# yifita/iso-points

Hardware: AMD Instinct MI355X
Metric: Mpoints/s full iso-point cycle (project+resample+splat), 1M pts (higher is better)
Workload: dtype f32-class (split-fp16 operands, 2^-22: hidden-layer products from two fp16 parts per f32 operand under exact power-of-two scales, 3 fp16-MFMA passes, f32 accumulate; everything else f32)

## Files before the change

### include/isopoints.h

```cpp
#ifndef ISOPOINTS_H_
#define ISOPOINTS_H_

#include <stdint.h>

#ifdef __cplusplus
extern "C" {
#endif

#define ISO_OK 0
#define ISO_ERR_INVALID (-1)
#define ISO_ERR_UNSUPPORTED (-2)
#define ISO_ERR_LAUNCH (-3)
#define ISO_ERR_WORKSPACE (-4)

const char* iso_version(void);
const char* iso_last_error(void);


int iso_project_sphere(const float* pts_in, float* pts_out, float* normals_out,
                       uint8_t* mask_out, int64_t n, float cx, float cy,
                       float cz, float radius, int max_iters, float tol,
                       void* stream);

typedef struct iso_follow {
  void* grid_ws; int64_t grid_n_max;
  const float* views; int n_views; float znear; float zfar; int backface_culling;
  int32_t* mask_out; void* front_ws; int64_t front_ws_bytes;
  int64_t* first_idx_out; int64_t* num_pts_out; int32_t* view_total_out;
} iso_follow;

int iso_project_sphere_follow(const float* pts_in, float* pts_out, float* normals_out,
                              uint8_t* mask_out, int64_t n, float cx, float cy,
                              float cz, float radius, int max_iters, float tol,
                              const iso_follow* follow_host, void* stream);

int64_t iso_siren_raw_floats(int hidden, int n_hidden);
int64_t iso_siren_packed_floats(int hidden, int n_hidden);
int iso_siren_pack_weights(const float* raw, float* packed, int hidden,
                           int n_hidden, void* stream);
int iso_siren_set_gemm_mode(int mode);
int iso_siren_get_gemm_mode(void);
int iso_siren_set_tail_from(int first_tail_iteration);
int iso_siren_set_drawn_tiles(int on);
int iso_idr_set_drawn_tiles(int on);
int iso_siren_step_launches(int hidden, int n_hidden, int max_iters);
int64_t iso_project_siren_workspace_bytes(int64_t n, int hidden, int n_hidden);
int64_t iso_project_siren_counts_offset(int64_t n, int hidden, int n_hidden);
int iso_project_siren(const float* pts_in, float* pts_out, float* normals_out,
                      uint8_t* mask_out, int64_t n, const float* packed,
                      int hidden, int n_hidden, float omega_first,
                      float omega_hidden, int max_iters, float tol,
                      void* workspace, int64_t workspace_bytes, void* stream);
int iso_siren_sdf_grad(const float* pts, float* sdf_out, float* grad_out,
                       int64_t n, const float* packed, int hidden,
                       int n_hidden, float omega_first, float omega_hidden,
                       void* workspace, int64_t workspace_bytes, void* stream);

int iso_siren_fold_codes(const float* w0c, const float* b0, const float* codes, float* table, int hidden,
                         int padded_hidden, int c_dim, int64_t n_codes, void* stream);
int iso_project_siren_coded(const float* pts_in, float* pts_out, float* normals_out,
                            uint8_t* mask_out, int64_t n, const float* packed,
                            int hidden, int n_hidden, float omega_first,
                            float omega_hidden, int max_iters, float tol,
                            void* workspace, int64_t workspace_bytes, void* stream,
                            const float* code_bias, const int32_t* code_of, int64_t n_codes);
int iso_siren_sdf_grad_coded(const float* pts, float* sdf_out, float* grad_out,
                             int64_t n, const float* packed, int hidden,
// ... 449 lines not shown
```

### iso_points_amd/_lib.py

```python
import ctypes
import os

import torch

_HERE = os.path.dirname(os.path.abspath(__file__))
LIB_PATH = os.path.join(_HERE, "libisopoints_hip.so")
if os.environ.get("ISO_DEV_LIB"):
    LIB_PATH = os.path.abspath(os.environ["ISO_DEV_LIB"])

_c = ctypes
_P = _c.c_void_p
_I = _c.c_int
_L = _c.c_int64
_F = _c.c_float

SIGNATURES = {
    "iso_version": (_c.c_char_p, []),
    "iso_last_error": (_c.c_char_p, []),
    "iso_project_sphere": (_I, [_P, _P, _P, _P, _L, _F, _F, _F, _F, _I, _F, _P]),
    "iso_project_sphere_follow": (_I, [_P, _P, _P, _P, _L, _F, _F, _F, _F, _I, _F, _P, _P]),
    "iso_siren_raw_floats": (_L, [_I, _I]),
    "iso_siren_packed_floats": (_L, [_I, _I]),
    "iso_siren_set_gemm_mode": (_I, [_I]),
    "iso_siren_get_gemm_mode": (_I, []),
    "iso_siren_set_tail_from": (_I, [_I]),
    "iso_siren_set_drawn_tiles": (_I, [_I]),
    "iso_idr_set_drawn_tiles": (_I, [_I]),
    "iso_siren_step_launches": (_I, [_I, _I, _I]),
    "iso_siren_pack_weights": (_I, [_P, _P, _I, _I, _P]),
    "iso_project_siren_workspace_bytes": (_L, [_L, _I, _I]),
    "iso_project_siren_counts_offset": (_L, [_L, _I, _I]),
    "iso_project_siren": (_I, [_P, _P, _P, _P, _L, _P, _I, _I, _F, _F, _I, _F, _P, _L, _P]),
    "iso_siren_sdf_grad": (_I, [_P, _P, _P, _L, _P, _I, _I, _F, _F, _P, _L, _P]),
    "iso_idr_set_gemm_mode": (_I, [_I]),
    "iso_idr_get_gemm_mode": (_I, []),
    "iso_idr_step_form": (_I, [_I, _I, _I, _I, _I]),
    "iso_idr_raw_floats": (_L, [_I, _I, _I, _I]),
    "iso_idr_packed_floats": (_L, [_I, _I]),
    "iso_idr_pack_weights": (_I, [_P, _P, _I, _I, _I, _I, _P]),
    "iso_project_idr_workspace_bytes": (_L, [_L, _I, _I]),
    "iso_project_idr": (_I, [_P, _P, _P, _P, _L, _P, _I, _I, _I, _I, _F, _I, _F, _P, _L, _P]),
    "iso_idr_sdf_grad": (_I, [_P, _P, _P, _L, _P, _I, _I, _I, _I, _F, _P, _L, _P]),
    "iso_trace_sphere": (_I, [_P, _P, _P, _P, _P, _L, _F, _F, _F, _F, _F, _F, _I, _F, _P]),
    "iso_trace_siren": (_I, [_P, _P, _P, _P, _P, _L, _P, _I, _I, _F, _F, _F, _F, _I, _F, _P, _L, _P]),
    "iso_siren_fold_codes": (_I, [_P, _P, _P, _P, _I, _I, _I, _L, _P]),
    "iso_project_siren_coded": (_I, [_P, _P, _P, _P, _L, _P, _I, _I, _F, _F, _I, _F, _P, _L, _P, _P, _P, _L]),
    "iso_siren_sdf_grad_coded": (_I, [_P, _P, _P, _L, _P, _I, _I, _F, _F, _P, _L, _P, _P, _P, _L]),
    "iso_trace_siren_coded": (_I, [_P, _P, _P, _P, _P, _L, _P, _I, _I, _F, _F, _F, _F, _I, _F, _P, _L, _P, _P, _P, _L]),
    "iso_trace_idr": (_I, [_P, _P, _P, _P, _P, _L, _P, _I, _I, _I, _I, _F, _F, _F, _I, _F, _P, _L, _P]),
    "iso_ray_nearest_point_workspace_bytes": (_L, [_L]),
# ... 181 lines not shown
```

### iso_points_amd/csrc/siren.hip

```cpp
#include <stdlib.h>
#include "siren_common.h"
#include "iso_newton.h"
#include "mlp_common.h"

namespace {

__global__ void k_siren_pack(const float* __restrict__ raw, float* __restrict__ packed,
                             int H, int L) {
  const int64_t total = off_hidden(H, L);
  const int64_t HH = (int64_t)H * H;
  const int NT = H / 16;
  for (int64_t o = (int64_t)blockIdx.x * blockDim.x + threadIdx.x; o < total;
       o += (int64_t)gridDim.x * blockDim.x) {
    float v = 0.f;
    if (o < off_wl(H)) {
      int64_t k = o;
      int c = (int)(k & 3);
      int e = (int)((k >> 2) % (H / 4));
      int g = (int)((k >> 2) / (H / 4));
      int f = 16 * (e >> 2) + 4 * g + (e & 3);
      v = (c < 3) ? raw[f * 3 + c] : raw[(int64_t)H * 3 + f];
    } else if (o < off_bl(H)) {
      int64_t k = o - off_wl(H);
      int e = (int)(k % (H / 4));
// ... 265 lines not shown
static int64_t tail_ints(int64_t n) { return siren_x3_tail_blocks() * (2 * tail_cap_of(n) + 2); }

constexpr int kTileCtrInts = 128;
extern "C" int64_t iso_project_siren_workspace_bytes(int64_t n, int hidden, int n_hidden) {
  if (n < 0) n = 0;
  return stash_floats_any(hidden, n_hidden) * 4 + 2 * n * 4 + tail_ints(n) * 4 + (64 + kTileCtrInts) * 4 + 64;
}

extern "C" int64_t iso_project_siren_counts_offset(int64_t n, int hidden, int n_hidden) {
  if (n < 0) n = 0;
  return stash_floats_any(hidden, n_hidden) * 4 + 2 * n * 4 + tail_ints(n) * 4;
}

static int g_siren_dyn_tiles = -1;
static bool siren_dynamic_tiles_enabled() {
  return g_siren_dyn_tiles != 0;
}
extern "C" int iso_siren_set_drawn_tiles(int on) {
  ISO_REQUIRE(on >= -1 && on <= 1, ISO_ERR_INVALID, "iso_siren_set_drawn_tiles: -1 (default), 0 or 1");
  g_siren_dyn_tiles = on;
  return ISO_OK;
}

static int run_step_split(SirenCodedArgs a, int hidden, int64_t n, hipStream_t s) {
  if (hidden == 256 && !a.fwd_only && use_x3(hidden, a.L)) {
    a.split = 3;
    return run_step(a, hidden, n, s);
  }
  a.split = 0;
  a.tile_ctr = nullptr;
  return run_step(a, hidden, n, s);
}

static int g_tail_from = -1;
static int siren_tail_from(int max_iters) {
  if (g_tail_from == 0) return max_iters + 1;
  if (g_tail_from > 0) return g_tail_from;
  return max_iters >= 6 ? 4 : 2;
}
extern "C" int iso_siren_step_launches(int hidden, int n_hidden, int max_iters) {
  if (max_iters < 0) return 0;
  const bool can_tail = hidden == 256 && use_x3(hidden, n_hidden);
  const int from = can_tail ? siren_tail_from(max_iters) : max_iters + 1;
  return from <= max_iters && from > 0 ? from + 1 : max_iters + 1;
}
extern "C" int iso_siren_set_tail_from(int first_tail_iteration) {
// ... 235 lines not shown
```

### iso_points_amd/csrc/siren_common.h

```cpp
#pragma once
#include "iso_common.h"

struct SirenArgs {
  float* pts;
  float* normals;
  uint8_t* mask;
  float* sdf_out;
  float* grad_out;
  const int32_t* idx_in;
  const int32_t* count_in;
  int32_t* idx_out;
  int32_t* count_out;
  const float* packed;
  float* stash;
  int64_t n;
  int L;
  float w0, wh, tol;
  int do_move;
  int eval_only;
  const float* dirs = nullptr;
  float alpha = 1.f, bound = 0.f, tol_valid = 0.f;
  int fwd_only = 0;
  int64_t cnt_lo = -1, cnt_hi = INT64_MAX;
  int small_tiles = 0;
// ... 28 lines not shown
__host__ __device__ inline int64_t off_hidden(int H, int l) {
  return 5 * (int64_t)H + 4 + (int64_t)l * ((int64_t)H + 2 * (int64_t)H * H);
}

__host__ __device__ inline int x3_feat(int s, int kappa) {
  return 32 * (s >> 1) + 16 * (s & 1) + 8 * ((kappa & 7) >> 2) + 4 * (kappa >> 3) + (kappa & 3);
}
__host__ __device__ inline int64_t x3_base(int H, int L) { return off_hidden(H, L); }
__host__ __device__ inline int64_t x3_off_w0(int H, int L) { return x3_base(H, L); }
__host__ __device__ inline int64_t x3_off_wl(int H, int L) { return x3_base(H, L) + 4 * (int64_t)H; }
__host__ __device__ inline int64_t x3_off_layer(int H, int L, int l) {
  return x3_base(H, L) + 5 * (int64_t)H + (int64_t)l * (int64_t)H;
}
constexpr int kX16Header = 24;
__host__ __device__ inline int64_t x16_base(int H, int L) { return x3_off_layer(H, L, L); }
__host__ __device__ inline int64_t x16_off_layer(int H, int L, int l) { return x16_base(H, L) + kX16Header + (int64_t)l * H * H; }
__host__ __device__ inline int64_t x16_off_bw(int H, int L, int l) { return x16_off_layer(H, L, L) + (int64_t)l * H * H; }
__host__ __device__ inline int64_t siren_packed_total(int H, int L) { return x16_off_bw(H, L, L); }

bool siren_x3_supported(int H, int L);
int64_t siren_x3_stash_floats(int H, int L);
void siren_x3_pack(const float* raw, float* packed, int H, int L, hipStream_t s);
int siren_x3_launch(const SirenCodedArgs& a, int H, int64_t n_upper, hipStream_t s);
int siren_x3_tail_blocks();
int siren_x3_launch_tail(const SirenCodedArgs& a, int H, hipStream_t s);
constexpr int64_t kPsMinList = 3 * 256 * 128;
__host__ __device__ inline bool siren_ps_takes(int64_t count, int L, const float* hdr , float wh) {
  if (count < kPsMinList) return false;
  float r = 0.f;
  for (int l = 0; l < L; ++l) r = hdr[17 + l] > r ? hdr[17 + l] : r;
  return (wh * r) * 1.01f < 1.0e4f;
}
```

### iso_points_amd/csrc/siren_x3.hip

```cpp
#include <stdlib.h>
#include <type_traits>
#include "siren_common.h"
#include "iso_newton.h"
#include "mlp_common.h"

#include "mfma_split.h"

constexpr int kAD = 3;

namespace {

__device__ __forceinline__ void x3_sin_wcos8(float w_in, float w, const float (&z)[8], float (&s)[8], float (&c)[8]) {
  iso_sin_wcos8(w_in, w, z, s, c);
}


__global__ void k_siren_pack_x3(const float* __restrict__ raw, float* __restrict__ packed, int H, int L) {
  const int64_t base = x3_base(H, L), total = x16_base(H, L);
  const int64_t HH = (int64_t)H * H;
  const float* b0 = raw + (int64_t)H * 3;
  const float* WL = raw + (int64_t)H * 4 + (int64_t)L * (HH + H);
  for (int64_t o = base + (int64_t)blockIdx.x * blockDim.x + threadIdx.x; o < total;
       o += (int64_t)gridDim.x * blockDim.x) {
    const int64_t rel = o - base;
// ... 77 lines not shown
    const bool bwd = o >= (int64_t)L * HH;
    const int l = (int)((o / HH) % L);
    const int64_t q = o % HH;
    const float* Wl = raw + (int64_t)H * 4 + (int64_t)l * (HH + H);
    const float sc = packed[x16_base(H, L) + l];
    const int d = (int)(q & 3), lane = (int)((q >> 2) & 63);
    const int64_t blk = q >> 8;
    const int part = (int)(blk & 1);
    const int To = (int)((blk >> 1) % NTO), s = (int)(blk / (2 * NTO));
    const int fo = 32 * To + (lane & 31);
    f32x2 v;
#pragma unroll
    for (int u = 0; u < 2; ++u) {
      const int fi = x3_feat(s, 8 * (lane >> 5) + 2 * d + u);
      v[u] = (bwd ? Wl[(int64_t)fi * H + fo] : Wl[(int64_t)fo * H + fi]) * sc;
    }
    const f16x2 h = __builtin_convertvector(v, f16x2);
    const f16x2 lo = __builtin_convertvector(v - __builtin_convertvector(h, f32x2), f16x2);
    reinterpret_cast<unsigned*>(packed + x16_off_layer(H, L, 0))[o] =
        part == 0 ? __builtin_bit_cast(unsigned, h) : __builtin_bit_cast(unsigned, lo);
  }
}

template <int H, int NW, int NB>
struct X3Shape {
  static constexpr int NS = H / 16;
  static constexpr int NTO = H / 32;
  static constexpr int TW = NTO / NW;
  static constexpr int SL = 2 * TW;
  static constexpr int NG = SL * NB;
  static constexpr int P = 32 * NB;
  static constexpr size_t kActBytes = (size_t)NS * NB * kAP * 1024;
  static constexpr size_t kRedBytes = (size_t)NW * P * 16;
  static constexpr size_t kPtsBytes = (size_t)P * 16;
  static constexpr int kLdsGroupsFit = (int)((163840 - (kActBytes + kRedBytes + kPtsBytes)) / ((size_t)NW * 2048));
  static constexpr int LG = kLdsGroupsFit < NG ? kLdsGroupsFit : NG;
  static constexpr size_t kLds = kActBytes + kRedBytes + kPtsBytes + (size_t)NW * LG * 2048;
  static constexpr int64_t kStashPerWg(int L) { return (int64_t)NW * (L > 1 ? L : 1) * NG * 512; }
  static_assert(NTO % NW == 0 && TW >= 1, "features must split evenly over the waves");
};

template <int H>
__device__ __forceinline__ void x3_code_bias8(const float* table, int row, int s, int h, float (&b)[8]) {
  const f32x4* t = reinterpret_cast<const f32x4*>(table + (int64_t)row * H + 16 * s + 4 * h);
  const f32x4 lo = t[0], hi = t[2];
#pragma unroll
  for (int e = 0; e < 4; ++e) { b[e] = lo[e]; b[4 + e] = hi[e]; }
}

template <int H, int NW, int NB, bool FWD, bool CODED>
__device__ __forceinline__ void x3_step_body(const typename SirenArgsOf<CODED>::type& a, const int bid, const int nblk,
                                             const int sid) {
  using S = X3Shape<H, NW, NB>;
  constexpr int NS = S::NS, NTO = S::NTO, TW = S::TW, SL = S::SL, NG = S::NG, P = S::P;
  extern __shared__ __attribute__((aligned(16))) unsigned char smem_raw[];
  u32x4* act = reinterpret_cast<u32x4*>(smem_raw);
  f32x4* red = reinterpret_cast<f32x4*>(smem_raw + S::kActBytes);
  f32x4* ptl = reinterpret_cast<f32x4*>(smem_raw + S::kActBytes + S::kRedBytes);
  constexpr int LG = S::LG;
  const int tid = threadIdx.x;
  const int w = __builtin_amdgcn_readfirstlane(tid >> 6);
  const int lane = tid & 63, h = lane >> 5, j = lane & 31;
  u32x4* own = act + (size_t)(SL * w) * NB * kAP * 64 + lane;
  u32x4* park = own + (size_t)(kAP - 2) * NG * 64;
  constexpr bool IL = (NW == 8);
  const int L = a.L;
  const float* X = a.packed + x3_base(H, L);
  const f32x4* W0u = reinterpret_cast<const f32x4*>(X) + SL * w * 16;
  const float* WLu = X + 4 * H + SL * w * 16;
  const int h8 = h * 8;
  const float bL = a.packed[off_bl(H)];
  f32x4* stash = reinterpret_cast<f32x4*>(a.stash) +
                 ((int64_t)sid * NW + w) * (int64_t)(L > 1 ? L : 1) * NG * 128;
  f32x4* lst = reinterpret_cast<f32x4*>(smem_raw + S::kActBytes + S::kRedBytes + S::kPtsBytes) + w * (LG * 128) + lane;

  constexpr int FP = 2, BP = 2;
  auto fwd_img = [&](int l) { return reinterpret_cast<const u32x4*>(a.packed + x16_off_layer(H, L, l)) + (TW * w * 2) * 64; };
  auto rev_img = [&](int l) { return reinterpret_cast<const u32x4*>(a.packed + x16_off_bw(H, L, l)) + (TW * w * 2) * 64; };
  auto fwd_scale = [&](int l) { return kActScale * a.packed[x16_base(H, L) + l]; };
  float* redm = reinterpret_cast<float*>(red);
  float bscale[NB];
  float amax[NB];
  auto put_amax = [&](int buf) {
#pragma unroll
    for (int n = 0; n < NB; ++n) {
      const float m = __builtin_fmaxf(amax[n], __shfl_xor(amax[n], 32));
      if (h == 0) redm[(buf * P + 32 * n + j) * NW + w] = m;
    }
  };
  u32x4 A[4][TW][3];
  x3_prefetch_a<kAD, TW, NTO, FP>(A, fwd_img(0), 0, lane);

  const int64_t total = a.count_in ? (int64_t)__hip_atomic_load(a.count_in, __ATOMIC_RELAXED, __HIP_MEMORY_SCOPE_AGENT) : a.n;
  if (total <= a.cnt_lo || total > a.cnt_hi) return;
  if (a.ps_guard && H == 256 && siren_ps_takes(total, L, a.packed + x16_base(H, L), a.wh)) return;
  const int64_t cut = a.split ? siren_split_point(total) : total;
  const int64_t slot0 = a.split == 2 ? cut : 0;
  const int64_t count = a.split == 1 ? cut : total;
  const int64_t n_tiles = (count - slot0 + P - 1) / P;
  __shared__ int s_next_tile, s_first_tile;
  int nidx[NB];
  float npx[NB], npy[NB], npz[NB];
  int nrow[NB];
  auto fetch_idx = [&](int64_t t) {
    int j_e = j;
    asm volatile("" : "+v"(j_e));
#pragma unroll
    for (int n = 0; n < NB; ++n) {
      const int64_t slot = slot0 + t * P + 32 * n + j_e;
      nidx[n] = -1;
      if (t < n_tiles && slot < count) nidx[n] = a.idx_in ? a.idx_in[slot] : (int)slot;
// ... 48 lines not shown
        float zz[8], hv[8], sv[8];
        if constexpr (CODED) {
          float bz[8];
          x3_code_bias8<H>(a.code_bias, row[n], SL * w + sl, h, bz);
#pragma unroll
          for (int e = 0; e < 8; ++e) zz[e] = ((wv[e].x * px[n] + wv[e].y * py[n]) + wv[e].z * pz[n]) + bz[e];
        } else {
#pragma unroll
          for (int e = 0; e < 8; ++e) zz[e] = ((wv[e].x * px[n] + wv[e].y * py[n]) + wv[e].z * pz[n]) + wv[e].w;
        }
        x3_sin_wcos8(a.w0, a.w0, zz, hv, sv);
        const int k = sl * NB + n;
        {
          u32x4 p0, p1;
          split8_f16(hv, p0, p1);
          own[(k * kAP + 0) * 64] = p0; own[(k * kAP + 1) * 64] = p1;
        }
        (void)sv;
      }
    }
    __syncthreads();

    f32x16 acc[TW][NB];
    float fpart[NB];
#pragma unroll
    for (int n = 0; n < NB; ++n) fpart[n] = 0.f;
    for (int l = 0; l < L; ++l) {
      const float* lay = a.packed + x3_off_layer(H, L, l);
      const u32x4* img = fwd_img(l);
      const float zscale = fwd_scale(l);
      const float w_in = a.wh / zscale;
      if (l + 1 < L || FWD) {
        gemm_x3<kAD, TW, NB, NTO, NS, kBias, IL, FP, FP>(img, lay, act + lane, acc, w, 0, A,
                                                         l + 1 < L ? fwd_img(l + 1) : fwd_img(0), 0, lane, zscale);
      } else {
        gemm_x3<kAD, TW, NB, NTO, NS, kBias, IL, FP, BP>(img, lay, act + lane, acc, w, 0, A, rev_img(L - 1), 0, lane,
                                                         zscale);
      }
      __syncthreads();
      const bool top = (l == L - 1);
      f32x4* st_l = stash + (int64_t)l * NG * 128;
      const bool lds_slot = (l == 0);
      const float seed_scale = x3_scale_for(a.packed[x16_base(H, L) + 16] * a.wh * 1.01f);
      if (top) {
#pragma unroll
        for (int n = 0; n < NB; ++n) { amax[n] = 0.f; bscale[n] = seed_scale; }
      }
      auto act_group = [&](int k, int n, int sl, const float (&zz)[8], float& fp) {
        float hv[8], sv[8];
        x3_sin_wcos8(w_in, a.wh, zz, hv, sv);
        if (top) {
          const f32x4 wl0 = *reinterpret_cast<const f32x4*>(WLu + sl * 16 + h8);
          const f32x4 wl1 = *reinterpret_cast<const f32x4*>(WLu + sl * 16 + h8 + 4);
          const float f0 = (wl0.x * hv[0] + wl0.y * hv[1]) + (wl0.z * hv[2] + wl0.w * hv[3]);
          const float f1 = (wl1.x * hv[4] + wl1.y * hv[5]) + (wl1.z * hv[6] + wl1.w * hv[7]);
          fp += f0 + f1;
          if constexpr (FWD) return;
#pragma unroll
          for (int e = 0; e < 4; ++e) { hv[e] = wl0[e] * sv[e]; hv[4 + e] = wl1[e] * sv[4 + e]; }
          float m = amax[n];
#pragma unroll
          for (int e = 0; e < 8; e += 2) m = __builtin_fmaxf(m, __builtin_fmaxf(__builtin_fabsf(hv[e]), __builtin_fabsf(hv[e + 1])));
          amax[n] = m;
          u32x4 p0, p1;
          split8_f16(hv, p0, p1, seed_scale);
          own[(k * kAP + 0) * 64] = p0; own[(k * kAP + 1) * 64] = p1;
          return;
        } else {
          if constexpr (!FWD) {
            if (k < LG && lds_slot) {
              lst[(k * 2 + 0) * 64] = (f32x4){sv[0], sv[1], sv[2], sv[3]};
              lst[(k * 2 + 1) * 64] = (f32x4){sv[4], sv[5], sv[6], sv[7]};
            } else {
              st_l[(k * 2 + 0) * 64 + lane] = (f32x4){sv[0], sv[1], sv[2], sv[3]};
              st_l[(k * 2 + 1) * 64 + lane] = (f32x4){sv[4], sv[5], sv[6], sv[7]};
            }
          }
        }
        u32x4 p0, p1;
        split8_f16(hv, p0, p1);
        own[(k * kAP + 0) * 64] = p0; own[(k * kAP + 1) * 64] = p1;
      };
      if constexpr (NG <= 8) {
#pragma unroll
        for (int t = 0; t < TW; ++t)
#pragma unroll
          for (int p = 0; p < 2; ++p)
#pragma unroll
            for (int n = 0; n < NB; ++n) {
              float zz[8];
#pragma unroll
              for (int e = 0; e < 8; ++e) zz[e] = acc[t][n][8 * p + e];
              act_group((2 * t + p) * NB + n, n, 2 * t + p, zz, fpart[n]);
              __builtin_amdgcn_sched_barrier(0);
            }
      } else {
#pragma unroll
        for (int t = 0; t < TW; ++t)
#pragma unroll
          for (int n = 0; n < NB; ++n)
#pragma unroll
            for (int p = 0; p < 2; ++p) {
              const int k = (2 * t + p) * NB + n;
              const f32x16& v = acc[t][n];
              park[(k * 2 + 0) * 64] = as_u32x4((f32x4){v[8 * p], v[8 * p + 1], v[8 * p + 2], v[8 * p + 3]});
              park[(k * 2 + 1) * 64] = as_u32x4((f32x4){v[8 * p + 4], v[8 * p + 5], v[8 * p + 6], v[8 * p + 7]});
            }
        for (int sl = 0; sl < SL; ++sl) {
          f32x4 z[NB][2];
#pragma unroll
          for (int n = 0; n < NB; ++n) {
            z[n][0] = as_f32x4(park[((sl * NB + n) * 2 + 0) * 64]);
            z[n][1] = as_f32x4(park[((sl * NB + n) * 2 + 1) * 64]);
          }
#pragma unroll
          for (int n = 0; n < NB; ++n) {
            float zz[8];
#pragma unroll
            for (int e = 0; e < 8; ++e) zz[e] = z[n][e >> 2][e & 3];
            act_group(sl * NB + n, n, sl, zz, fpart[n]);
          }
        }
      }
      if constexpr (!FWD) { if (top) put_amax(0); }
      __syncthreads();
    }
    float gx[NB], gy[NB], gz[NB];
#pragma unroll
    for (int n = 0; n < NB; ++n) gx[n] = gy[n] = gz[n] = 0.f;
    int mbuf = 0;
    auto get_amax = [&](float (&Mp)[NB]) {
#pragma unroll
      for (int n = 0; n < NB; ++n) {
        float m = 0.f;
#pragma unroll
        for (int ww = 0; ww < NW; ++ww) m = __builtin_fmaxf(m, redm[(mbuf * P + 32 * n + j) * NW + ww]);
        Mp[n] = m;
      }
    };
    for (int l = FWD ? 0 : L - 1; l >= 1; --l) {
      const u32x4* img = rev_img(l);
      const f32x4* st_l = stash + (int64_t)(l - 1) * NG * 128;
      f32x4 sv[NG][2];
      auto ld_stash = [&]() {
#pragma unroll
        for (int k = 0; k < NG; ++k) {
          if (k < LG && l == 1) {
            sv[k][0] = lst[(k * 2) * 64]; sv[k][1] = lst[(k * 2 + 1) * 64];
          } else {
            sv[k][0] = st_l[(k * 2) * 64 + lane]; sv[k][1] = st_l[(k * 2 + 1) * 64 + lane];
          }
        }
      };
      float Mp[NB];
      get_amax(Mp);
      gemm_x3<kAD, TW, NB, NTO, NS, kZero, IL, BP, BP>(img, nullptr, act + lane, acc, w, 0, A, rev_img(l - 1), 0, lane);
      ld_stash();
      __syncthreads();
      float inv[NB], nscale[NB];
      {
        const float iw = 1.0f / a.packed[x16_base(H, L) + l];
        const float grow = a.packed[x16_base(H, L) + 8 + l] * a.wh * 1.01f;
#pragma unroll
        for (int n = 0; n < NB; ++n) {
          inv[n] = iw / bscale[n];
          nscale[n] = x3_scale_for(Mp[n] * grow);
          amax[n] = 0.f;
        }
      }
#pragma unroll
      for (int t = 0; t < TW; ++t)
#pragma unroll
        for (int p = 0; p < 2; ++p) {
#pragma unroll
          for (int n = 0; n < NB; ++n) {
            const int k = (2 * t + p) * NB + n;
            float av[8];
#pragma unroll
            for (int e = 0; e < 8; ++e) av[e] = (acc[t][n][8 * p + e] * inv[n]) * sv[k][e >> 2][e & 3];
            float m = amax[n];
#pragma unroll
            for (int e = 0; e < 8; e += 2) m = __builtin_fmaxf(m, __builtin_fmaxf(__builtin_fabsf(av[e]), __builtin_fabsf(av[e + 1])));
            amax[n] = m;
            u32x4 p0, p1;
            split8_f16(av, p0, p1, nscale[n]);
            own[(k * kAP + 0) * 64] = p0; own[(k * kAP + 1) * 64] = p1;
          }
        }
#pragma unroll
      for (int n = 0; n < NB; ++n) bscale[n] = nscale[n];
      put_amax(mbuf ^ 1);
      mbuf ^= 1;
      __syncthreads();
    }
    if constexpr (!FWD) {
      int drawn = 0;
      if (dyn && tid == 0) drawn = draw_base + atomicAdd(a.tile_ctr, 1);
      gemm_x3<kAD, TW, NB, NTO, NS, kZero, IL, BP, FP>(rev_img(0), nullptr, act + lane, acc, w, 0, A, fwd_img(0), 0, lane);
      if (dyn && tid == 0) s_next_tile = drawn;
      __syncthreads();
      next_tile = dyn ? (int64_t)s_next_tile : tile + nblk;
      fetch_idx(next_tile);
      float inv[NB];
      {
        const float iw = 1.0f / a.packed[x16_base(H, L)];
#pragma unroll
        for (int n = 0; n < NB; ++n) inv[n] = iw / bscale[n];
      }
      f32x4 q[NB];
#pragma unroll
      for (int n = 0; n < NB; ++n) q[n] = ptl[32 * n + j];
#pragma unroll
      for (int t = 0; t < TW; ++t)
#pragma unroll
        for (int p = 0; p < 2; ++p) {
          f32x4 wv[8];
#pragma unroll
          for (int e = 0; e < 8; ++e) wv[e] = W0u[(2 * t + p) * 16 + h8 + e];
#pragma unroll
          for (int n = 0; n < NB; ++n) {
            float zz[8], cv[8];
            if constexpr (CODED) {
              float bz[8];
              x3_code_bias8<H>(a.code_bias, __float_as_int(q[n].w), SL * w + 2 * t + p, h, bz);
#pragma unroll
              for (int e = 0; e < 8; ++e) zz[e] = ((wv[e].x * q[n].x + wv[e].y * q[n].y) + wv[e].z * q[n].z) + bz[e];
            } else {
#pragma unroll
              for (int e = 0; e < 8; ++e) zz[e] = ((wv[e].x * q[n].x + wv[e].y * q[n].y) + wv[e].z * q[n].z) + wv[e].w;
            }
            iso_wcos8(a.w0, a.w0, zz, cv);
#pragma unroll
            for (int e = 0; e < 8; ++e) {
              const float av = (acc[t][n][8 * p + e] * inv[n]) * cv[e];
              gx[n] += wv[e].x * av;
              gy[n] += wv[e].y * av;
              gz[n] += wv[e].z * av;
            }
            __builtin_amdgcn_sched_barrier(0);
          }
        }
    } else {
      next_tile = tile + nblk;
      fetch_idx(next_tile);
    }
#pragma unroll
    for (int n = 0; n < NB; ++n) {
      float f = fpart[n] + __shfl_xor(fpart[n], 32);
      float x = gx[n] + __shfl_xor(gx[n], 32);
      float y = gy[n] + __shfl_xor(gy[n], 32);
      float z = gz[n] + __shfl_xor(gz[n], 32);
      if (h == 0) red[w * P + 32 * n + j] = (f32x4){f, x, y, z};
    }
    int tid_e = tid, lane_e = lane;
    asm volatile("" : "+v"(tid_e), "+v"(lane_e));
    int eidx = -1;
    f32x4 qe = {0.f, 0.f, 0.f, 0.f};
    {
      const int64_t slot = slot0 + tile * P + tid_e;
      if (tid_e < P && slot < count) {
        eidx = a.idx_in ? a.idx_in[slot] : (int)slot;
        if constexpr (!FWD) qe = ptl[tid_e];
      }
      fetch_pts();
    }
    __syncthreads();
    bool survive = false;
    int64_t idx = -1;
    {
      const int64_t slot = slot0 + tile * P + tid_e;
      if (tid_e < P && slot < count) {
        f32x4 r = red[tid_e];
#pragma unroll
        for (int ww = 1; ww < NW; ++ww) {
          const f32x4 q = red[ww * P + tid_e];
          r.x += q.x; r.y += q.y; r.z += q.z; r.w += q.w;
        }
        const float f = r.x + bL;
        idx = eidx;
        if constexpr (!FWD) survive = iso_step_finish<SirenArgs, true>(a, idx, f, r.y, r.z, r.w, qe.x, qe.y, qe.z);
        else survive = iso_step_finish(a, idx, f, r.y, r.z, r.w);
      }
    }
    if (!a.eval_only && a.do_move) {
      const unsigned long long bal = __ballot(survive);
      if (bal) {
        int base = 0;
        const int leader = __ffsll((long long)bal) - 1;
        if (lane_e == leader) base = atomicAdd(a.count_out, __popcll(bal));
        base = __shfl(base, leader);
        if (survive) {
          const int rank = __popcll(bal & ((1ull << lane_e) - 1ull));
          a.idx_out[base + rank] = (int32_t)idx;
        }
      }
    }
  }
}
// ... 5 lines not shown

template <int H, int NW, int NB, int MINB, bool CODED>
__global__ __launch_bounds__(64 * NW, MINB) void k_siren_step_x3_both(typename SirenArgsOf<CODED>::type a) {
  const bool big = (int)blockIdx.x < a.big_blocks;
  const int small_blocks = (int)gridDim.x - a.big_blocks;
  if (big) {
    typename SirenArgsOf<CODED>::type b = a;
    b.split = 1;
    x3_step_body<H, NW, NB, false, CODED>(b, (int)blockIdx.x, a.big_blocks, (int)blockIdx.x);
  }
  if (!big || a.tile_ctr != nullptr) {
    if (big) __syncthreads();
    typename SirenArgsOf<CODED>::type b = a;
    b.split = 2;
    if (a.tile_ctr) b.tile_ctr = a.tile_ctr + 1;
    const bool joint = a.tile_ctr != nullptr;
    b.draw_first = joint ? 1 : 0;
    const int bid = big ? small_blocks + (int)blockIdx.x : (int)blockIdx.x - a.big_blocks;
    const int nblk = joint ? small_blocks + a.big_blocks : small_blocks;
    if (big) b.stash = a.stash + (int64_t)blockIdx.x * X3Shape<H, NW, NB>::kStashPerWg(a.L);
    else b.stash = a.stash + (int64_t)a.big_blocks * X3Shape<H, NW, NB>::kStashPerWg(a.L);
    x3_step_body<H, NW, 1, false, CODED>(b, bid, nblk, big ? 0 : bid);
  }
}

template <int H, int NW, int MINB, bool CODED>
__global__ __launch_bounds__(64 * NW, MINB) void k_siren_tail_x3(typename SirenArgsOf<CODED>::type a) {
  const int b = blockIdx.x, nblk = gridDim.x;
  int32_t* lists = a.tail_lists + (int64_t)b * 2 * a.tail_cap;
  int32_t* cnts = a.tail_counts + b * 2;
  typename SirenArgsOf<CODED>::type r = a;
  r.split = 0; r.small_tiles = 1; r.cnt_lo = -1; r.cnt_hi = INT64_MAX; r.tile_ctr = nullptr;
  r.idx_out = lists; r.count_out = cnts;
  r.do_move = a.it_first < a.it_last ? 1 : 0;
  x3_step_body<H, NW, 1, false, CODED>(r, b, nblk, b);
  int cur = 0;
  for (int it = a.it_first + 1; it <= a.it_last; ++it) {
    __syncthreads();
    const int m = __hip_atomic_load(&cnts[cur], __ATOMIC_RELAXED, __HIP_MEMORY_SCOPE_AGENT);
    if (m == 0) break;
    if (threadIdx.x == 0) {
      __hip_atomic_store(&cnts[cur ^ 1], 0, __ATOMIC_RELAXED, __HIP_MEMORY_SCOPE_AGENT);
      if (a.iter_counts) atomicAdd(&a.iter_counts[it], m);
    }
    __syncthreads();
    r.idx_in = lists + (int64_t)cur * a.tail_cap; r.count_in = cnts + cur;
    r.idx_out = lists + (int64_t)(cur ^ 1) * a.tail_cap; r.count_out = cnts + (cur ^ 1);
    r.do_move = it < a.it_last ? 1 : 0;
    x3_step_body<H, NW, 1, false, CODED>(r, 0, 1, b);
    cur ^= 1;
  }
  __syncthreads();
  if (threadIdx.x == 0) { cnts[0] = 0; cnts[1] = 0; }
}

template <int H, int NW, int NB, int MINB, bool FWD, bool CODED>
int launch_x3(const typename SirenArgsOf<CODED>::type& a, int64_t n_upper, hipStream_t s) {
  using S = X3Shape<H, NW, NB>;
  static bool attr_done = false;
  if (!attr_done) {
    (void)hipFuncSetAttribute(reinterpret_cast<const void*>(&k_siren_step_x3<H, NW, NB, MINB, FWD, CODED>),
                              hipFuncAttributeMaxDynamicSharedMemorySize, (int)S::kLds);
    attr_done = true;
  }
  const int64_t tiles = (n_upper + S::P - 1) / S::P;
  const int64_t cap = 256 * MINB;
  const int blocks = (int)(tiles < cap ? (tiles < 1 ? 1 : tiles) : cap);
  hipLaunchKernelGGL((k_siren_step_x3<H, NW, NB, MINB, FWD, CODED>), dim3(blocks), dim3(64 * NW), S::kLds, s, a);
  return 0;
}

template <int H, int NW, int NB, int MINB, bool CODED>
int launch_x3_both(typename SirenArgsOf<CODED>::type a, int64_t n_upper, hipStream_t s) {
  using SB = X3Shape<H, NW, NB>;
  using SS = X3Shape<H, NW, 1>;
  constexpr size_t lds = SB::kLds > SS::kLds ? SB::kLds : SS::kLds;
  static bool attr_done = false;
  if (!attr_done) {
    (void)hipFuncSetAttribute(reinterpret_cast<const void*>(&k_siren_step_x3_both<H, NW, NB, MINB, CODED>),
                              hipFuncAttributeMaxDynamicSharedMemorySize, (int)lds);
    attr_done = true;
  }
  const int64_t cap = 256 * MINB;
  const int64_t tb = (n_upper + SB::P - 1) / SB::P, ts = (n_upper + SS::P - 1) / SS::P;
  a.big_blocks = (int)(tb < cap ? (tb < 1 ? 1 : tb) : cap);
  const int small_blocks = (int)(ts < cap ? (ts < 1 ? 1 : ts) : cap);
  hipLaunchKernelGGL((k_siren_step_x3_both<H, NW, NB, MINB, CODED>), dim3(a.big_blocks + small_blocks), dim3(64 * NW), lds, s, a);
  return 0;
}

}

constexpr int kNW256 = 8;
constexpr int kMinB256 = 1;
constexpr int kNB256 = 3;
constexpr int kMinB128 = 1;
bool siren_x3_supported(int H, int L) { return (H == 256 || H == 128) && L >= 1 && L <= 8; }

int64_t siren_x3_stash_floats(int H, int L) {
  if (H == 256) {
    return 256 * kMinB256 * (X3Shape<256, kNW256, kNB256>::kStashPerWg(L) + X3Shape<256, kNW256, 1>::kStashPerWg(L));
  }
  if (H == 128) return 256 * kMinB128 * X3Shape<128, 4, 3>::kStashPerWg(L);
  return 0;
}

void siren_x3_pack(const float* raw, float* packed, int H, int L, hipStream_t s) {
  const int64_t words = x16_base(H, L) - x3_base(H, L);
  hipLaunchKernelGGL(k_siren_pack_x3, dim3(iso_stream_grid(words, 256)), dim3(256), 0, s, raw, packed, H, L);
  if (L > 0) {
// ... 2 lines not shown
  }
}

int siren_x3_tail_blocks() { return 256 * kMinB256; }

template <bool CODED>
static int launch_tail(const typename SirenArgsOf<CODED>::type& a, hipStream_t s) {
  using SS = X3Shape<256, kNW256, 1>;
  static bool attr_done = false;
  if (!attr_done) {
    (void)hipFuncSetAttribute(reinterpret_cast<const void*>(&k_siren_tail_x3<256, kNW256, kMinB256, CODED>),
                              hipFuncAttributeMaxDynamicSharedMemorySize, (int)SS::kLds);
    attr_done = true;
  }
  hipLaunchKernelGGL((k_siren_tail_x3<256, kNW256, kMinB256, CODED>), dim3(siren_x3_tail_blocks()), dim3(64 * kNW256), SS::kLds, s, a);
  return 0;
}

int siren_x3_launch_tail(const SirenCodedArgs& a, int H, hipStream_t s) {
  if (H != 256) return -1;
  return a.code_bias ? launch_tail<true>(a, s) : launch_tail<false>(a, s);
}

template <bool CODED>
static int launch_any(const typename SirenArgsOf<CODED>::type& a, int H, int64_t n_upper, hipStream_t s) {
  if (a.split == 3 && H == 256 && !a.fwd_only) return launch_x3_both<256, kNW256, kNB256, kMinB256, CODED>(a, n_upper, s);
  if (a.fwd_only) {
    if (H == 256) return launch_x3<256, kNW256, kNB256, kMinB256, true, CODED>(a, n_upper, s);
    if (H == 128) return launch_x3<128, 4, 3, kMinB128, true, CODED>(a, n_upper, s);
  }
  if constexpr (!CODED) {
    if (H == 256) return launch_x3<256, kNW256, kNB256, kMinB256, false, false>(a, n_upper, s);
  }
  if (H == 128) return launch_x3<128, 4, 3, kMinB128, false, CODED>(a, n_upper, s);
  return -1;
}

int siren_x3_launch(const SirenCodedArgs& a, int H, int64_t n_upper, hipStream_t s) {
  return a.code_bias ? launch_any<true>(a, H, n_upper, s) : launch_any<false>(a, H, n_upper, s);
}
```

Measured before the change: 77.14.

## Add four-wave SIREN step form keeping activation stash in registers and LDS

```diff
diff --git a/include/isopoints.h b/include/isopoints.h
--- a/include/isopoints.h
+++ b/include/isopoints.h
@@ -43,6 +43,9 @@
 int iso_siren_set_tail_from(int first_tail_iteration);
 int iso_siren_set_drawn_tiles(int on);
 int iso_idr_set_drawn_tiles(int on);
+int iso_siren_set_step_form(int form);
+int iso_siren_get_step_form(void);
+int iso_siren_step_form_used(int hidden, int n_hidden, int coded);
 int iso_siren_step_launches(int hidden, int n_hidden, int max_iters);
 int64_t iso_project_siren_workspace_bytes(int64_t n, int hidden, int n_hidden);
 int64_t iso_project_siren_counts_offset(int64_t n, int hidden, int n_hidden);
diff --git a/iso_points_amd/_lib.py b/iso_points_amd/_lib.py
--- a/iso_points_amd/_lib.py
+++ b/iso_points_amd/_lib.py
@@ -26,6 +26,9 @@
     "iso_siren_set_tail_from": (_I, [_I]),
     "iso_siren_set_drawn_tiles": (_I, [_I]),
     "iso_idr_set_drawn_tiles": (_I, [_I]),
+    "iso_siren_set_step_form": (_I, [_I]),
+    "iso_siren_get_step_form": (_I, []),
+    "iso_siren_step_form_used": (_I, [_I, _I, _I]),
     "iso_siren_step_launches": (_I, [_I, _I, _I]),
     "iso_siren_pack_weights": (_I, [_P, _P, _I, _I, _P]),
     "iso_project_siren_workspace_bytes": (_L, [_L, _I, _I]),
diff --git a/iso_points_amd/csrc/siren.hip b/iso_points_amd/csrc/siren.hip
--- a/iso_points_amd/csrc/siren.hip
+++ b/iso_points_amd/csrc/siren.hip
@@ -311,6 +311,16 @@
   return ISO_OK;
 }
 
+extern "C" int iso_siren_set_step_form(int form) {
+  ISO_REQUIRE(form == 0 || form == 1, ISO_ERR_INVALID, "iso_siren_set_step_form: 0 (eight waves, global stash) or 1 (four waves, stash on chip)");
+  siren_x3_set_step_form(form);
+  return ISO_OK;
+}
+extern "C" int iso_siren_get_step_form(void) { return siren_x3_get_step_form(); }
+extern "C" int iso_siren_step_form_used(int hidden, int n_hidden, int coded) {
+  return use_x3(hidden, n_hidden) && siren_x3_on_chip(hidden, n_hidden, false, coded != 0) ? 1 : 0;
+}
+
 static int run_step_split(SirenCodedArgs a, int hidden, int64_t n, hipStream_t s) {
   if (hidden == 256 && !a.fwd_only && use_x3(hidden, a.L)) {
     a.split = 3;
diff --git a/iso_points_amd/csrc/siren_common.h b/iso_points_amd/csrc/siren_common.h
--- a/iso_points_amd/csrc/siren_common.h
+++ b/iso_points_amd/csrc/siren_common.h
@@ -74,6 +74,9 @@
 int64_t siren_x3_stash_floats(int H, int L);
 void siren_x3_pack(const float* raw, float* packed, int H, int L, hipStream_t s);
 int siren_x3_launch(const SirenCodedArgs& a, int H, int64_t n_upper, hipStream_t s);
+void siren_x3_set_step_form(int form);
+int siren_x3_get_step_form();
+bool siren_x3_on_chip(int H, int L, bool fwd_only, bool coded);
 int siren_x3_tail_blocks();
 int siren_x3_launch_tail(const SirenCodedArgs& a, int H, hipStream_t s);
 constexpr int64_t kPsMinList = 3 * 256 * 128;
diff --git a/iso_points_amd/csrc/siren_x3.hip b/iso_points_amd/csrc/siren_x3.hip
--- a/iso_points_amd/csrc/siren_x3.hip
+++ b/iso_points_amd/csrc/siren_x3.hip
@@ -123,7 +123,7 @@
   }
 }
 
-template <int H, int NW, int NB>
+template <int H, int NW, int NB, int RP = 1>
 struct X3Shape {
   static constexpr int NS = H / 16;
   static constexpr int NTO = H / 32;
@@ -132,13 +132,14 @@
   static constexpr int NG = SL * NB;
   static constexpr int P = 32 * NB;
   static constexpr size_t kActBytes = (size_t)NS * NB * kAP * 1024;
-  static constexpr size_t kRedBytes = (size_t)NW * P * 16;
+  static constexpr size_t kRedBytes = RP > 1 ? (size_t)2 * P * NW * 4 : (size_t)NW * P * 16;
   static constexpr size_t kPtsBytes = (size_t)P * 16;
   static constexpr int kLdsGroupsFit = (int)((163840 - (kActBytes + kRedBytes + kPtsBytes)) / ((size_t)NW * 2048));
   static constexpr int LG = kLdsGroupsFit < NG ? kLdsGroupsFit : NG;
   static constexpr size_t kLds = kActBytes + kRedBytes + kPtsBytes + (size_t)NW * LG * 2048;
   static constexpr int64_t kStashPerWg(int L) { return (int64_t)NW * (L > 1 ? L : 1) * NG * 512; }
   static_assert(NTO % NW == 0 && TW >= 1, "features must split evenly over the waves");
+  static_assert(RP == 1 || (size_t)NW * LG * 2048 >= (size_t)NW * RP * P * 16, "the final reduction fits the LDS stash");
 };
 
 template <int H>
@@ -149,10 +150,13 @@
   for (int e = 0; e < 4; ++e) { b[e] = lo[e]; b[4 + e] = hi[e]; }
 }
 
-template <int H, int NW, int NB, bool FWD, bool CODED>
+template <int H, int NW, int NB, bool FWD, bool CODED, int LT = 0>
 __device__ __forceinline__ void x3_step_body(const typename SirenArgsOf<CODED>::type& a, const int bid, const int nblk,
                                              const int sid) {
-  using S = X3Shape<H, NW, NB>;
+  constexpr bool RS = LT > 0;
+  constexpr int RP = RS ? (H / 32) / NW : 1;
+  static_assert(!RS || !FWD, "the on-chip form is a gradient kernel");
+  using S = X3Shape<H, NW, NB, RP>;
   constexpr int NS = S::NS, NTO = S::NTO, TW = S::TW, SL = S::SL, NG = S::NG, P = S::P;
   extern __shared__ __attribute__((aligned(16))) unsigned char smem_raw[];
   u32x4* act = reinterpret_cast<u32x4*>(smem_raw);
@@ -164,8 +168,8 @@
   const int lane = tid & 63, h = lane >> 5, j = lane & 31;
   u32x4* own = act + (size_t)(SL * w) * NB * kAP * 64 + lane;
   u32x4* park = own + (size_t)(kAP - 2) * NG * 64;
-  constexpr bool IL = (NW == 8);
-  const int L = a.L;
+  constexpr bool IL = (NW == 8) || RS;
+  const int L = RS ? LT : a.L;
   const float* X = a.packed + x3_base(H, L);
   const f32x4* W0u = reinterpret_cast<const f32x4*>(X) + SL * w * 16;
   const float* WLu = X + 4 * H + SL * w * 16;
@@ -174,6 +178,7 @@
   f32x4* stash = reinterpret_cast<f32x4*>(a.stash) +
                  ((int64_t)sid * NW + w) * (int64_t)(L > 1 ? L : 1) * NG * 128;
   f32x4* lst = reinterpret_cast<f32x4*>(smem_raw + S::kActBytes + S::kRedBytes + S::kPtsBytes) + w * (LG * 128) + lane;
+  f32x4* redf = RS ? reinterpret_cast<f32x4*>(smem_raw + S::kActBytes + S::kRedBytes + S::kPtsBytes) : red;
 
   constexpr int FP = 2, BP = 2;
   auto fwd_img = [&](int l) { return reinterpret_cast<const u32x4*>(a.packed + x16_off_layer(H, L, l)) + (TW * w * 2) * 64; };
@@ -188,6 +193,11 @@
       const float m = __builtin_fmaxf(amax[n], __shfl_xor(amax[n], 32));
       if (h == 0) redm[(buf * P + 32 * n + j) * NW + w] = m;
     }
+  };
+  auto stage_lane = [&]() __attribute__((always_inline)) {
+    int v = lane;
+    if constexpr (RS) asm volatile("" : "+v"(v));
+    return v;
   };
   u32x4 A[4][TW][3];
   x3_prefetch_a<kAD, TW, NTO, FP>(A, fwd_img(0), 0, lane);
@@ -282,19 +292,24 @@
     __syncthreads();
 
     f32x16 acc[TW][NB];
-    float fpart[NB];
-#pragma unroll
-    for (int n = 0; n < NB; ++n) fpart[n] = 0.f;
-    for (int l = 0; l < L; ++l) {
+    f32x4 rst[RS && LT > 1 ? LT - 1 : 1][RS ? NG : 1][2];
+    float fpart[RP][NB];
+#pragma unroll
+    for (int r = 0; r < RP; ++r)
+#pragma unroll
+      for (int n = 0; n < NB; ++n) fpart[r][n] = 0.f;
+    auto fwd_layer = [&](auto lc) __attribute__((always_inline)) {
+      const int l = lc;
+      const int gl = stage_lane();
       const float* lay = a.packed + x3_off_layer(H, L, l);
       const u32x4* img = fwd_img(l);
       const float zscale = fwd_scale(l);
       const float w_in = a.wh / zscale;
       if (l + 1 < L || FWD) {
-        gemm_x3<kAD, TW, NB, NTO, NS, kBias, IL, FP, FP>(img, lay, act + lane, acc, w, 0, A,
-                                                         l + 1 < L ? fwd_img(l + 1) : fwd_img(0), 0, lane, zscale);
+        gemm_x3<kAD, TW, NB, NTO, NS, kBias, IL, FP, FP>(img, lay, act + gl, acc, w, 0, A,
+                                                         l + 1 < L ? fwd_img(l + 1) : fwd_img(0), 0, gl, zscale);
       } else {
-        gemm_x3<kAD, TW, NB, NTO, NS, kBias, IL, FP, BP>(img, lay, act + lane, acc, w, 0, A, rev_img(L - 1), 0, lane,
+        gemm_x3<kAD, TW, NB, NTO, NS, kBias, IL, FP, BP>(img, lay, act + gl, acc, w, 0, A, rev_img(L - 1), 0, gl,
                                                          zscale);
       }
       __syncthreads();
@@ -315,6 +330,7 @@
           const float f0 = (wl0.x * hv[0] + wl0.y * hv[1]) + (wl0.z * hv[2] + wl0.w * hv[3]);
           const float f1 = (wl1.x * hv[4] + wl1.y * hv[5]) + (wl1.z * hv[6] + wl1.w * hv[7]);
           fp += f0 + f1;
+          if constexpr (RS) asm volatile("" : "+v"(fp));
           if constexpr (FWD) return;
 #pragma unroll
           for (int e = 0; e < 4; ++e) { hv[e] = wl0[e] * sv[e]; hv[4 + e] = wl1[e] * sv[4 + e]; }
@@ -331,6 +347,11 @@
             if (k < LG && lds_slot) {
               lst[(k * 2 + 0) * 64] = (f32x4){sv[0], sv[1], sv[2], sv[3]};
               lst[(k * 2 + 1) * 64] = (f32x4){sv[4], sv[5], sv[6], sv[7]};
+            } else if constexpr (RS) {
+              if constexpr (LT > 1) {
+                rst[l < LT - 1 ? l : 0][k][0] = (f32x4){sv[0], sv[1], sv[2], sv[3]};
+                rst[l < LT - 1 ? l : 0][k][1] = (f32x4){sv[4], sv[5], sv[6], sv[7]};
+              }
             } else {
               st_l[(k * 2 + 0) * 64 + lane] = (f32x4){sv[0], sv[1], sv[2], sv[3]};
               st_l[(k * 2 + 1) * 64 + lane] = (f32x4){sv[4], sv[5], sv[6], sv[7]};
@@ -341,7 +362,7 @@
         split8_f16(hv, p0, p1);
         own[(k * kAP + 0) * 64] = p0; own[(k * kAP + 1) * 64] = p1;
       };
-      if constexpr (NG <= 8) {
+      if constexpr (NG <= 8 || RS) {
 #pragma unroll
         for (int t = 0; t < TW; ++t)
 #pragma unroll
@@ -351,7 +372,7 @@
               float zz[8];
 #pragma unroll
               for (int e = 0; e < 8; ++e) zz[e] = acc[t][n][8 * p + e];
-              act_group((2 * t + p) * NB + n, n, 2 * t + p, zz, fpart[n]);
+              act_group((2 * t + p) * NB + n, n, 2 * t + p, zz, fpart[RS ? t : 0][n]);
               __builtin_amdgcn_sched_barrier(0);
             }
       } else {
@@ -378,16 +399,26 @@
             float zz[8];
 #pragma unroll
             for (int e = 0; e < 8; ++e) zz[e] = z[n][e >> 2][e & 3];
-            act_group(sl * NB + n, n, sl, zz, fpart[n]);
+            act_group(sl * NB + n, n, sl, zz, fpart[0][n]);
           }
         }
       }
       if constexpr (!FWD) { if (top) put_amax(0); }
       __syncthreads();
-    }
-    float gx[NB], gy[NB], gz[NB];
-#pragma unroll
-    for (int n = 0; n < NB; ++n) gx[n] = gy[n] = gz[n] = 0.f;
+    };
+    if constexpr (RS) {
+      static_assert(LT <= 3, "layers are expanded by hand");
+      fwd_layer(std::integral_constant<int, 0>());
+      if constexpr (LT > 1) fwd_layer(std::integral_constant<int, 1>());
+      if constexpr (LT > 2) fwd_layer(std::integral_constant<int, 2>());
+    } else {
+      for (int l = 0; l < L; ++l) fwd_layer(l);
+    }
+    float gx[RP][NB], gy[RP][NB], gz[RP][NB];
+#pragma unroll
+    for (int r = 0; r < RP; ++r)
+#pragma unroll
+      for (int n = 0; n < NB; ++n) gx[r][n] = gy[r][n] = gz[r][n] = 0.f;
     int mbuf = 0;
     auto get_amax = [&](float (&Mp)[NB]) {
 #pragma unroll
@@ -398,7 +429,9 @@
         Mp[n] = m;
       }
     };
-    for (int l = FWD ? 0 : L - 1; l >= 1; --l) {
+    auto rev_stage = [&](auto lc) __attribute__((always_inline)) {
+      const int l = lc;
+      const int gl = stage_lane();
       const u32x4* img = rev_img(l);
       const f32x4* st_l = stash + (int64_t)(l - 1) * NG * 128;
       f32x4 sv[NG][2];
@@ -407,6 +440,8 @@
         for (int k = 0; k < NG; ++k) {
           if (k < LG && l == 1) {
             sv[k][0] = lst[(k * 2) * 64]; sv[k][1] = lst[(k * 2 + 1) * 64];
+          } else if constexpr (RS) {
+            if constexpr (LT > 1) { sv[k][0] = rst[l - 1 < LT - 1 ? l - 1 : 0][k][0]; sv[k][1] = rst[l - 1 < LT - 1 ? l - 1 : 0][k][1]; }
           } else {
             sv[k][0] = st_l[(k * 2) * 64 + lane]; sv[k][1] = st_l[(k * 2 + 1) * 64 + lane];
           }
@@ -414,7 +449,7 @@
       };
       float Mp[NB];
       get_amax(Mp);
-      gemm_x3<kAD, TW, NB, NTO, NS, kZero, IL, BP, BP>(img, nullptr, act + lane, acc, w, 0, A, rev_img(l - 1), 0, lane);
+      gemm_x3<kAD, TW, NB, NTO, NS, kZero, IL, BP, BP>(img, nullptr, act + gl, acc, w, 0, A, rev_img(l - 1), 0, gl);
       ld_stash();
       __syncthreads();
       float inv[NB], nscale[NB];
@@ -445,6 +480,7 @@
             u32x4 p0, p1;
             split8_f16(av, p0, p1, nscale[n]);
             own[(k * kAP + 0) * 64] = p0; own[(k * kAP + 1) * 64] = p1;
+            if constexpr (RS) __builtin_amdgcn_sched_barrier(0);
           }
         }
 #pragma unroll
@@ -452,11 +488,18 @@
       put_amax(mbuf ^ 1);
       mbuf ^= 1;
       __syncthreads();
+    };
+    if constexpr (RS) {
+      if constexpr (LT > 2) rev_stage(std::integral_constant<int, 2>());
+      if constexpr (LT > 1) rev_stage(std::integral_constant<int, 1>());
+    } else {
+      for (int l = FWD ? 0 : L - 1; l >= 1; --l) rev_stage(l);
     }
     if constexpr (!FWD) {
+      const int gl = stage_lane();
       int drawn = 0;
       if (dyn && tid == 0) drawn = draw_base + atomicAdd(a.tile_ctr, 1);
-      gemm_x3<kAD, TW, NB, NTO, NS, kZero, IL, BP, FP>(rev_img(0), nullptr, act + lane, acc, w, 0, A, fwd_img(0), 0, lane);
+      gemm_x3<kAD, TW, NB, NTO, NS, kZero, IL, BP, FP>(rev_img(0), nullptr, act + gl, acc, w, 0, A, fwd_img(0), 0, gl);
       if (dyn && tid == 0) s_next_tile = drawn;
       __syncthreads();
       next_tile = dyn ? (int64_t)s_next_tile : tile + nblk;
@@ -493,9 +536,9 @@
 #pragma unroll
             for (int e = 0; e < 8; ++e) {
               const float av = (acc[t][n][8 * p + e] * inv[n]) * cv[e];
-              gx[n] += wv[e].x * av;
-              gy[n] += wv[e].y * av;
-              gz[n] += wv[e].z * av;
+              gx[RS ? t : 0][n] += wv[e].x * av;
+              gy[RS ? t : 0][n] += wv[e].y * av;
+              gz[RS ? t : 0][n] += wv[e].z * av;
             }
             __builtin_amdgcn_sched_barrier(0);
           }
@@ -505,12 +548,14 @@
       fetch_idx(next_tile);
     }
 #pragma unroll
+    for (int r = 0; r < RP; ++r)
+#pragma unroll
     for (int n = 0; n < NB; ++n) {
-      float f = fpart[n] + __shfl_xor(fpart[n], 32);
-      float x = gx[n] + __shfl_xor(gx[n], 32);
-      float y = gy[n] + __shfl_xor(gy[n], 32);
-      float z = gz[n] + __shfl_xor(gz[n], 32);
-      if (h == 0) red[w * P + 32 * n + j] = (f32x4){f, x, y, z};
+      float f = fpart[r][n] + __shfl_xor(fpart[r][n], 32);
+      float x = gx[r][n] + __shfl_xor(gx[r][n], 32);
+      float y = gy[r][n] + __shfl_xor(gy[r][n], 32);
+      float z = gz[r][n] + __shfl_xor(gz[r][n], 32);
+      if (h == 0) redf[(RP * w + r) * P + 32 * n + j] = (f32x4){f, x, y, z};
     }
     int tid_e = tid, lane_e = lane;
     asm volatile("" : "+v"(tid_e), "+v"(lane_e));
@@ -530,10 +575,10 @@
     {
       const int64_t slot = slot0 + tile * P + tid_e;
       if (tid_e < P && slot < count) {
-        f32x4 r = red[tid_e];
-#pragma unroll
-        for (int ww = 1; ww < NW; ++ww) {
-          const f32x4 q = red[ww * P + tid_e];
+        f32x4 r = redf[tid_e];
+#pragma unroll
+        for (int ww = 1; ww < NW * RP; ++ww) {
+          const f32x4 q = redf[ww * P + tid_e];
           r.x += q.x; r.y += q.y; r.z += q.z; r.w += q.w;
         }
         const float f = r.x + bL;
@@ -585,6 +630,37 @@
     else b.stash = a.stash + (int64_t)a.big_blocks * X3Shape<H, NW, NB>::kStashPerWg(a.L);
     x3_step_body<H, NW, 1, false, CODED>(b, bid, nblk, big ? 0 : bid);
   }
+}
+
+constexpr int kOcNW = 4;
+template <int H, int NB, int MINB, bool CODED, int LT>
+__global__ __launch_bounds__(64 * kOcNW, MINB) void k_siren_step_x3_oc(typename SirenArgsOf<CODED>::type a) {
+  x3_step_body<H, kOcNW, NB, false, CODED, LT>(a, (int)blockIdx.x, (int)gridDim.x, (int)blockIdx.x);
+}
+template <int H, int NB, bool CODED, int LT>
+__device__ __forceinline__ void x3_both_oc(const typename SirenArgsOf<CODED>::type& a) {
+  const bool big = (int)blockIdx.x < a.big_blocks;
+  const int small_blocks = (int)gridDim.x - a.big_blocks;
+  if (big) {
+    typename SirenArgsOf<CODED>::type b = a;
+    b.split = 1;
+    x3_step_body<H, kOcNW, NB, false, CODED, LT>(b, (int)blockIdx.x, a.big_blocks, (int)blockIdx.x);
+  }
+  if (!big || a.tile_ctr != nullptr) {
+    if (big) __syncthreads();
+    typename SirenArgsOf<CODED>::type b = a;
+    b.split = 2;
+    if (a.tile_ctr) b.tile_ctr = a.tile_ctr + 1;
+    const bool joint = a.tile_ctr != nullptr;
+    b.draw_first = joint ? 1 : 0;
+    const int bid = big ? small_blocks + (int)blockIdx.x : (int)blockIdx.x - a.big_blocks;
+    const int nblk = joint ? small_blocks + a.big_blocks : small_blocks;
+    x3_step_body<H, kOcNW, 1, false, CODED, LT>(b, bid, nblk, big ? 0 : bid);
+  }
+}
+template <int H, int NB, int MINB, bool CODED, int LT>
+__global__ __launch_bounds__(64 * kOcNW, MINB) void k_siren_step_x3_both_oc(typename SirenArgsOf<CODED>::type a) {
+  x3_both_oc<H, NB, CODED, LT>(a);
 }
 
 template <int H, int NW, int MINB, bool CODED>
@@ -617,38 +693,47 @@
   if (threadIdx.x == 0) { cnts[0] = 0; cnts[1] = 0; }
 }
 
-template <int H, int NW, int NB, int MINB, bool FWD, bool CODED>
+template <int H, int NW, int NB, int MINB, bool FWD, bool CODED, int LT = 0>
 int launch_x3(const typename SirenArgsOf<CODED>::type& a, int64_t n_upper, hipStream_t s) {
-  using S = X3Shape<H, NW, NB>;
+  using S = X3Shape<H, NW, NB, (LT > 0 ? (H / 32) / NW : 1)>;
+  static_assert(LT == 0 || (NW == kOcNW && !FWD), "the on-chip form: four waves, gradient kernels");
+  static_assert(S::kLds <= 163840, "LDS of a gfx950 CU");
+  void (*kern)(typename SirenArgsOf<CODED>::type);
+  if constexpr (LT > 0) kern = &k_siren_step_x3_oc<H, NB, MINB, CODED, LT>;
+  else kern = &k_siren_step_x3<H, NW, NB, MINB, FWD, CODED>;
   static bool attr_done = false;
   if (!attr_done) {
-    (void)hipFuncSetAttribute(reinterpret_cast<const void*>(&k_siren_step_x3<H, NW, NB, MINB, FWD, CODED>),
-                              hipFuncAttributeMaxDynamicSharedMemorySize, (int)S::kLds);
+    (void)hipFuncSetAttribute(reinterpret_cast<const void*>(kern), hipFuncAttributeMaxDynamicSharedMemorySize, (int)S::kLds);
     attr_done = true;
   }
   const int64_t tiles = (n_upper + S::P - 1) / S::P;
   const int64_t cap = 256 * MINB;
   const int blocks = (int)(tiles < cap ? (tiles < 1 ? 1 : tiles) : cap);
-  hipLaunchKernelGGL((k_siren_step_x3<H, NW, NB, MINB, FWD, CODED>), dim3(blocks), dim3(64 * NW), S::kLds, s, a);
+  hipLaunchKernelGGL(kern, dim3(blocks), dim3(64 * NW), S::kLds, s, a);
   return 0;
 }
 
-template <int H, int NW, int NB, int MINB, bool CODED>
+template <int H, int NW, int NB, int MINB, bool CODED, int LT = 0>
 int launch_x3_both(typename SirenArgsOf<CODED>::type a, int64_t n_upper, hipStream_t s) {
-  using SB = X3Shape<H, NW, NB>;
-  using SS = X3Shape<H, NW, 1>;
+  constexpr int RP = LT > 0 ? (H / 32) / NW : 1;
+  using SB = X3Shape<H, NW, NB, RP>;
+  using SS = X3Shape<H, NW, 1, RP>;
+  static_assert(LT == 0 || NW == kOcNW, "the on-chip form: four waves");
   constexpr size_t lds = SB::kLds > SS::kLds ? SB::kLds : SS::kLds;
+  static_assert(lds <= 163840, "LDS of a gfx950 CU");
+  void (*kern)(typename SirenArgsOf<CODED>::type);
+  if constexpr (LT > 0) kern = &k_siren_step_x3_both_oc<H, NB, MINB, CODED, LT>;
+  else kern = &k_siren_step_x3_both<H, NW, NB, MINB, CODED>;
   static bool attr_done = false;
   if (!attr_done) {
-    (void)hipFuncSetAttribute(reinterpret_cast<const void*>(&k_siren_step_x3_both<H, NW, NB, MINB, CODED>),
-                              hipFuncAttributeMaxDynamicSharedMemorySize, (int)lds);
+    (void)hipFuncSetAttribute(reinterpret_cast<const void*>(kern), hipFuncAttributeMaxDynamicSharedMemorySize, (int)lds);
     attr_done = true;
   }
   const int64_t cap = 256 * MINB;
   const int64_t tb = (n_upper + SB::P - 1) / SB::P, ts = (n_upper + SS::P - 1) / SS::P;
   a.big_blocks = (int)(tb < cap ? (tb < 1 ? 1 : tb) : cap);
   const int small_blocks = (int)(ts < cap ? (ts < 1 ? 1 : ts) : cap);
-  hipLaunchKernelGGL((k_siren_step_x3_both<H, NW, NB, MINB, CODED>), dim3(a.big_blocks + small_blocks), dim3(64 * NW), lds, s, a);
+  hipLaunchKernelGGL(kern, dim3(a.big_blocks + small_blocks), dim3(64 * NW), lds, s, a);
   return 0;
 }
 
@@ -697,8 +782,25 @@
   return a.code_bias ? launch_tail<true>(a, s) : launch_tail<false>(a, s);
 }
 
+static int g_step_form = 1;
+void siren_x3_set_step_form(int form) { g_step_form = form; }
+int siren_x3_get_step_form() { return g_step_form; }
+bool siren_x3_on_chip(int H, int L, bool fwd_only, bool coded) {
+  return g_step_form == 1 && H == 256 && (L == 2 || L == 3) && !fwd_only && !coded;
+}
+
 template <bool CODED>
 static int launch_any(const typename SirenArgsOf<CODED>::type& a, int H, int64_t n_upper, hipStream_t s) {
+  if constexpr (!CODED) {
+    if (siren_x3_on_chip(H, a.L, a.fwd_only != 0, false)) {
+      if (a.split == 3) {
+        return a.L == 3 ? launch_x3_both<256, kOcNW, kNB256, kMinB256, false, 3>(a, n_upper, s)
+                        : launch_x3_both<256, kOcNW, kNB256, kMinB256, false, 2>(a, n_upper, s);
+      }
+      return a.L == 3 ? launch_x3<256, kOcNW, kNB256, kMinB256, false, false, 3>(a, n_upper, s)
+                      : launch_x3<256, kOcNW, kNB256, kMinB256, false, false, 2>(a, n_upper, s);
+    }
+  }
   if (a.split == 3 && H == 256 && !a.fwd_only) return launch_x3_both<256, kNW256, kNB256, kMinB256, CODED>(a, n_upper, s);
   if (a.fwd_only) {
     if (H == 256) return launch_x3<256, kNW256, kNB256, kMinB256, true, CODED>(a, n_upper, s);
```

Result: faster. 89.06, median of 6 (+15.5%).
